# ka9q/ka9q-radio

Hardware: NVIDIA H100
Metric: input Msamples/s through forward+filter+inverse at N channels (higher is better)
Workload: dtype f32

## Files before the change

ka9q_radio_b200/csrc/fft_static.cuh:

```cuda
#pragma once
#include "fft_radix.cuh"

namespace kfft {

template <int LEN, int... RS> struct SPlan {
  static constexpr int len = LEN;
  static constexpr int nst = sizeof...(RS);
  static constexpr int rad_arr[sizeof...(RS) > 0 ? sizeof...(RS) : 1] = {RS...};
  static constexpr int rad(int i) { return rad_arr[i]; }
  static constexpr int nsub(int i) {
    int n = LEN;
    for (int k = 0; k < i; k++) n /= rad_arr[k];
    return n;
  }
  static constexpr int stride(int i) { return nsub(i) / rad_arr[i]; }
  static constexpr int tw_off(int i) {
    int o = 0;
    for (int k = 0; k < i; k++)
      if (stride(k) > 1) o += (rad_arr[k] - 1) * stride(k);
    return o;
  }
  static constexpr bool valid() {
    int p = 1;
    for (int k = 0; k < nst; k++) p *= rad_arr[k];
    return p == LEN;
  }
};

template <class P, int I = 0> struct SlotOf {
  static __device__ __forceinline__ int run(int rem) {
    constexpr int R = P::rad(I), S = P::stride(I);
    int const q = rem / R;
    return (rem - q * R) * S + SlotOf<P, I + 1>::run(q);
  }
};
template <class P> struct SlotOf<P, P::nst> {
  static __device__ __forceinline__ int run(int) { return 0; }
};
template <class P> __device__ __forceinline__ int static_slot(int k) { return SlotOf<P>::run(k); }

template <class P> constexpr int static_tw_count() { return P::tw_off(P::nst); }

__device__ __forceinline__ int ldg_stream_b32(int const *p) {
  int v;
  asm volatile("ld.global.nc.L1::no_allocate.b32 %0, [%1];" : "=r"(v) : "l"(p));
  return v;
}
__device__ __forceinline__ float2 ldg_stream_f2(float2 const *p) {
  float2 v;
  asm volatile("ld.global.nc.L1::no_allocate.v2.f32 {%0, %1}, [%2];" : "=f"(v.x), "=f"(v.y) : "l"(p));
  return v;
}

template <class P, int I> struct StageGeom {
  static constexpr int R = P::rad(I), NSUB = P::nsub(I), S = P::stride(I), NB = P::len / R;
  static __device__ __forceinline__ void split(int u, int &b, int &j) {
    if (S == 1) {
      b = u;
      j = 0;
    } else {
      b = u / S;
      j = u - b * S;
    }
  }
};

template <class P, bool INV, int I, bool TWS, int ILP>
__device__ __forceinline__ void static_stage(float2 *__restrict__ col, float2 const *__restrict__ tw, int lane) {
  using G = StageGeom<P, I>;
  constexpr int R = G::R, NSUB = G::NSUB, S = G::S, NB = G::NB, NL = 32;
  constexpr int ITERS = (NB + NL - 1) / NL;
  float2 const *twi = tw + P::tw_off(I);
#pragma unroll
  for (int it0 = 0; it0 < ITERS; it0 += ILP) {
    float2 x[ILP][R];
    float2 *p[ILP];
    int jj[ILP];
    bool ok[ILP];
#pragma unroll
    for (int q = 0; q < ILP; q++) {
      int const u = lane + NL * (it0 + q);
      ok[q] = (it0 + q < ITERS) && ((NB % NL == 0) || it0 + q + 1 < ITERS || u < NB);
      int b, j;
      G::split(ok[q] ? u : 0, b, j);
      jj[q] = j;
      p[q] = col + b * NSUB + j;
      if (ok[q]) {
#pragma unroll
        for (int m = 0; m < R; m++) x[q][m] = p[q][m * S];
      }
    }
#pragma unroll
    for (int q = 0; q < ILP; q++) {
      if (ok[q]) {
        Dft<R, INV>::run(x[q]);
        if (S > 1) {
#pragma unroll
          for (int t = 1; t < R; t++) {
            float2 const w = TWS ? twi[(t - 1) * S + jj[q]] : __ldg(twi + (t - 1) * S + jj[q]);
            x[q][t] = INV ? cmulc(x[q][t], w) : cmul(x[q][t], w);
          }
        }
      }
    }
#pragma unroll
    for (int q = 0; q < ILP; q++) {
      if (ok[q]) {
#pragma unroll
        for (int t = 0; t < R; t++) p[q][t * S] = x[q][t];
      }
    }
  }
}

template <class P, bool INV, bool TWS = false, int ILP = 1, int I = 0> struct StaticFft {
  static __device__ __forceinline__ void run(float2 *col, float2 const *tw, int lane) {
    static_stage<P, INV, I, TWS, (P::rad(I) <= 12 ? ILP : 1)>(col, tw, lane);
    __syncwarp();
    StaticFft<P, INV, TWS, ILP, I + 1>::run(col, tw, lane);
  }
};
template <class P, bool INV, bool TWS, int ILP> struct StaticFft<P, INV, TWS, ILP, P::nst> {
  static __device__ __forceinline__ void run(float2 *, float2 const *, int) {}
};

__device__ __forceinline__ uint32_t smem_u32(void const *p) { return (uint32_t)__cvta_generic_to_shared(p); }
__device__ __forceinline__ void mbar_init(uint64_t *bar, int count) {
  asm volatile("mbarrier.init.shared::cta.b64 [%0], %1;" ::"r"(smem_u32(bar)), "r"(count));
}
__device__ __forceinline__ void mbar_fence_init() { asm volatile("fence.mbarrier_init.release.cluster;" ::: "memory"); }
__device__ __forceinline__ void mbar_expect_tx(uint64_t *bar, uint32_t bytes) {
  asm volatile("mbarrier.arrive.expect_tx.shared::cta.b64 _, [%0], %1;" ::"r"(smem_u32(bar)), "r"(bytes) : "memory");
}
__device__ __forceinline__ void bulk_g2s(void *dst, void const *src, uint32_t bytes, uint64_t *bar) {
  asm volatile("cp.async.bulk.shared::cluster.global.mbarrier::complete_tx::bytes [%0], [%1], %2, [%3];" ::"r"(smem_u32(dst)),
               "l"(src), "r"(bytes), "r"(smem_u32(bar))
               : "memory");
}
__device__ __forceinline__ void tensor_g2s_3d(void *dst, void const *map, int x, int y, int z, uint64_t *bar) {
  asm volatile("cp.async.bulk.tensor.3d.shared::cluster.global.tile.mbarrier::complete_tx::bytes [%0], [%1, {%2, %3, %4}], [%5];"
               ::"r"(smem_u32(dst)), "l"(map), "r"(x), "r"(y), "r"(z), "r"(smem_u32(bar))
               : "memory");
}
__device__ __forceinline__ void fence_proxy_async_global() { asm volatile("fence.proxy.async.global;" ::: "memory"); }
__device__ __forceinline__ void discard_l2_line(void *p) { asm volatile("discard.global.L2 [%0], 128;" ::"l"(p) : "memory"); }
__device__ __forceinline__ void mbar_wait(uint64_t *bar, uint32_t parity) {
  asm volatile(
      "{\n\t.reg .pred p;\n\t"
      "WAIT_%=:\n\t"
      "mbarrier.try_wait.parity.shared::cta.b64 p, [%0], %1;\n\t"
      "@p bra DONE_%=;\n\t"
      "bra WAIT_%=;\n\t"
      "DONE_%=:\n\t}" ::"r"(smem_u32(bar)),
      "r"(parity)
      : "memory");
}

}
```

ka9q_radio_b200/csrc/fwd_fused.cuh:

```cuda
#pragma once
#include "fwd_cols_r36.cuh"
#include "static_kernels_v2.cuh"

namespace kfft {

struct FusedShape {
  static constexpr int N1 = 1296, N2 = 1250;
  static constexpr int TILES = (N2 + 7) / 8;
  static constexpr int NC = (TILES + 1) / 2;
  static constexpr int NR = (N1 / 2 + 1 + RowsV2Shape<true>::IPC - 1) / RowsV2Shape<true>::IPC;
  static constexpr int T = 2 * ColsR36Shape::T;
  static constexpr int RT = RowsV2Shape<true>::T;
  static constexpr size_t smem = 2 * ColsR36Shape::smem > RowsV2Shape<true>::smem ? 2 * ColsR36Shape::smem : RowsV2Shape<true>::smem;
  static constexpr int DEFAULT_LEAD = 40;
  static_assert(ColsR36Shape::smem % 16 == 0, "the second tile's memory 16-byte aligned");
  static_assert(T % 32 == 0 && ColsR36Shape::T % 32 == 0 && RT % 32 == 0, "whole warps per tile and per R item");
};

enum FusedKind : int { kFusedCol = 0, kFusedRow = 1 };
struct FusedItem {
  int kind, blk, idx;
};

__host__ __device__ __forceinline__ FusedItem fused_item(int t, int nblocks, int lead) {
  using F = FusedShape;
  if (t < F::NC) return {kFusedCol, 0, t};
  t -= F::NC;
  int const b = t / (F::NR + F::NC), p = t - b * (F::NR + F::NC);
  if (b >= nblocks - 1) return {kFusedRow, nblocks - 1, t - (nblocks - 1) * (F::NR + F::NC)};
  if (p < lead) return {kFusedCol, b + 1, p};
  int const q = p - lead, m = F::NC - lead;
  if (q < 2 * m) return (q & 1) ? FusedItem{kFusedCol, b + 1, lead + q / 2} : FusedItem{kFusedRow, b, q / 2};
  return {kFusedRow, b, q - m};
}

struct FusedArgs {
  unsigned *ctr;
  int nblocks, lead;
  int discard;
};

__device__ __forceinline__ void red_release_gpu_add(unsigned *p, unsigned v) {
  asm volatile("red.release.gpu.global.add.u32 [%0], %1;" ::"l"(p), "r"(v) : "memory");
}
__device__ __forceinline__ unsigned ld_acquire_gpu(unsigned const *p) {
  unsigned v;
  asm volatile("ld.acquire.gpu.global.u32 %0, [%1];" : "=r"(v) : "l"(p) : "memory");
  return v;
}

template <int FMT>
__global__ void __launch_bounds__(FusedShape::T, 1)
    fwd_fused_r36_v2(Pass1Args const a1, ColsR36Tables const t1, Pass2Args const a2, FwdTables const t2, FusedArgs const f,
                     const __grid_constant__ CUtensorMap tmap) {
  using F = FusedShape;
  extern __shared__ __align__(16) unsigned char smem_raw[];
  __shared__ __align__(8) uint64_t bars[RowsV2Shape<true>::COLS];
  __shared__ __align__(8) uint64_t tbar[2];
  __shared__ int s_ticket;
  int const tid = threadIdx.x;
  if (tid == 0) s_ticket = (int)atomicAdd(f.ctr, 1u);
  __syncthreads();
  FusedItem const it = fused_item(s_ticket, f.nblocks, f.lead);
  if (it.kind == kFusedCol) {
    int const h = tid >= ColsR36Shape::T, tile = 2 * it.idx + h;
    if (tile < F::TILES)
      fwd_cols_r36_body<FMT, F::N2, true>(a1, t1, &tmap, smem_raw + h * ColsR36Shape::smem, tbar[h], tid - h * ColsR36Shape::T,
                                           tile * 8, it.blk, [h] {
                                             asm volatile("bar.sync %0, %1;" ::"r"(1 + h), "n"(ColsR36Shape::T) : "memory");
                                           });
    __syncthreads();
    if (tid == 0) {
      __threadfence();
      red_release_gpu_add(f.ctr + 1 + fused_item(s_ticket, f.nblocks, f.lead).blk, 1u);
    }
    return;
  }
  if (tid >= F::RT) return;
  auto sync = [] { asm volatile("bar.sync 3, %0;" ::"n"(F::RT) : "memory"); };
  auto sync_or = [](int p) {
    int r;
    asm volatile("{\n\t.reg .pred q, o;\n\tsetp.ne.s32 q, %1, 0;\n\tbar.red.or.pred o, 3, %2, q;\n\tselp.s32 %0, 1, 0, o;\n\t}"
                 : "=r"(r)
                 : "r"(p), "n"(F::RT)
                 : "memory");
    return r;
  };
  if (tid == 0)
    while (ld_acquire_gpu(f.ctr + 1 + it.blk) < (unsigned)F::NC) __nanosleep(64);
  sync();
  fwd_rows_v2_body<true, F::N1, true, true>(a2, t2, smem_raw, bars, tbar[0], tid, it.blk, it.idx * RowsV2Shape<true>::IPC,
                                            sync, sync_or, f.discard);
}

}
```

ka9q_radio_b200/csrc/static_kernels_v2.cuh:

```cuda
#pragma once
#include "static_kernels.cuh"

namespace kfft {

__device__ __forceinline__ void unpack_i16(int raw, int &lo, int &hi) {
  asm("prmt.b32 %0, %1, 0, 0x9910;" : "=r"(lo) : "r"(raw));
  hi = raw >> 16;
}
__device__ __forceinline__ float i32_to_f32(int v) {
  float f;
  asm("cvt.rn.f32.s32 %0, %1;" : "=f"(f) : "r"(v));
  return f;
}

template <bool REAL_SPLIT>
struct RowsV2Shape {
  using P = SPlan<1250, 10, 25, 5>;
  static constexpr int N2 = 1250, PITCH = 1250, GT = 256, SKEW = 2;
  static constexpr int NG = REAL_SPLIT ? 2 : 1, T = GT * NG, COLS = 8 * NG;
  static constexpr int IPC = REAL_SPLIT ? COLS / 2 : COLS;
  static constexpr int TW = (static_tw_count<P>() + 1) & ~1;
  static constexpr int TILE = COLS * PITCH + (NG - 1) * SKEW;
  static constexpr size_t smem = sizeof(float2) * (size_t)(TILE + TW);
  static __host__ __device__ constexpr int col_off(int c) { return c * PITCH + (c >> 3) * SKEW; }
};

__device__ constexpr float kRowsTw0[3][4][2] = {
    {{9.870916009e-01f, -1.601568460e-01f}, {9.486995935e-01f, -3.161789477e-01f}, {8.000617623e-01f, -5.999176502e-01f}, {2.801976204e-01f, -9.599423409e-01f}},
    {{9.486995935e-01f, -3.161789477e-01f}, {8.000617623e-01f, -5.999176502e-01f}, {2.801976204e-01f, -9.599423409e-01f}, {-8.429785967e-01f, -5.379471183e-01f}},
    {{8.858151436e-01f, -4.640382826e-01f}, {5.693368912e-01f, -8.221042752e-01f}, {-3.517109454e-01f, -9.361086488e-01f}, {-7.525988221e-01f, 6.584793329e-01f}},
};

__host__ __device__ constexpr int mid_row_lines(int mid_ld) { return mid_ld * 8 / 128; }
__host__ __device__ constexpr long mid_line(int blk, int n1, int row, int mid_ld, int l) {
  return ((long)blk * n1 + row) * mid_row_lines(mid_ld) + l;
}

template <bool REAL_SPLIT, int N1C, bool HALVED, bool FUSED, class Sync, class SyncOr>
__device__ __forceinline__ void fwd_rows_v2_body(Pass2Args const &a, FwdTables const &tb, unsigned char *smem_raw,
                                                 uint64_t *bars, uint64_t &tbar, int tid, int blk, int item0,
                                                 Sync const &sync, SyncOr const &sync_or, bool discard = false) {
  using S = RowsV2Shape<REAL_SPLIT>;
  using P = typename S::P;
  constexpr int N2 = S::N2, T = S::T, GT = S::GT, COLS = S::COLS, IPC = S::IPC;
  constexpr int R0 = 10, S0 = 125, R1 = 25, NSUB1 = 125, S1 = 5, R2 = 5;
  float2 *tile = reinterpret_cast<float2 *>(smem_raw);
  float2 *s_tw = tile + S::TILE;
  TilePlan const &pl = c_plans[a.plan];
  int const lane = tid & 31, warp = tid >> 5;
  int const n1 = N1C ? N1C : a.n1;
  auto row_of = [&](int col) -> int {
    RowItem const it = row_item(item0 + (REAL_SPLIT ? col >> 1 : col), n1, REAL_SPLIT);
    if (REAL_SPLIT) {
      if ((col & 1) == 0) return it.kind != kRowEmpty ? it.row_a : -1;
      return it.kind == kRowPair ? it.row_b : -1;
    }
    return it.kind == kRowPlain ? it.row_a : -1;
  };
  if (lane == 0) {
    int const row = row_of(warp);
    mbar_init(&bars[warp], 1);
    if (warp == 0) mbar_init(&tbar, 1);
    mbar_fence_init();
    if (row >= 0) {
      if (FUSED) fence_proxy_async_global();
      mbar_expect_tx(&bars[warp], N2 * 8);
      bulk_g2s(tile + S::col_off(warp), a.mid + ((long)blk * n1 + row) * a.mid_ld, N2 * 8, &bars[warp]);
    }
    if (warp == 0) {
      constexpr uint32_t TWB = (uint32_t)S::TW * 8u;
      mbar_expect_tx(&tbar, TWB);
      bulk_g2s(s_tw, pl.tw, TWB, &tbar);
    }
  }
  sync();
  int const g = tid / GT;
  int const c = (tid & 7) + 8 * g, ul = (tid % GT) >> 3;
  auto group_sync = [&] {
    if (S::NG == 1) sync();
    else asm volatile("bar.sync %0, %1;" ::"r"(1 + g), "n"(GT) : "memory");
  };
  bool const col_ok = row_of(c) >= 0;
  mbar_wait(&tbar, 0);
  if (col_ok) mbar_wait(&bars[c], 0);
  if (FUSED && discard && col_ok) {
    char *const mid = const_cast<char *>(reinterpret_cast<char const *>(a.mid));
    for (int l = ul; l < mid_row_lines(a.mid_ld); l += GT / 8) discard_l2_line(mid + 128 * mid_line(blk, n1, row_of(c), a.mid_ld, l));
  }
  float2 *mycol = tile + S::col_off(c);

  if (col_ok) {
    float2 base[4];
#pragma unroll
    for (int q = 0; q < 4; q++) base[q] = s_tw[((1 << q) - 1) * S0 + ul];
#pragma unroll
    for (int it = 0; it < 4; it++) {
      int const j = ul + (GT / 8) * it;
      if (it < 3 || j < S0) {
        float2 *p = mycol + j;
        float2 x[R0], w[R0];
#pragma unroll
        for (int m = 0; m < R0; m++) x[m] = p[m * S0];
#pragma unroll
        for (int q = 0; q < 4; q++)
          w[1 << q] = it == 0 ? base[q] : cmul(base[q], make_float2(kRowsTw0[it > 0 ? it - 1 : 0][q][0], kRowsTw0[it > 0 ? it - 1 : 0][q][1]));
        w[3] = cmul(w[2], w[1]);
        w[5] = cmul(w[4], w[1]);
        w[6] = cmul(w[4], w[2]);
        w[7] = cmul(w[4], w[3]);
        w[9] = cmul(w[8], w[1]);
        Dft<R0, false>::run(x);
        p[0] = x[0];
#pragma unroll
        for (int t = 1; t < R0; t++) p[t * S0] = cmul(x[t], w[t]);
      }
    }
  }
  group_sync();
  if (col_ok) {
    float2 const *tw1 = s_tw + P::tw_off(1);
#pragma unroll 1
    for (int u = ul; u < N2 / R1; u += GT / 8) {
      int const b = u / S1, j = u - b * S1;
      float2 *p = mycol + b * NSUB1 + j;
      float2 x[R1];
#pragma unroll
      for (int m = 0; m < R1; m++) x[m] = p[m * S1];
      Dft<R1, false>::run(x);
#pragma unroll
      for (int t = 1; t < R1; t++) x[t] = cmul(x[t], tw1[(t - 1) * S1 + j]);
#pragma unroll
      for (int t = 0; t < R1; t++) p[t * S1] = x[t];
    }
  }
  constexpr int UQ = T / IPC;
  int const i = tid % IPC, uq = tid / IPC;
  RowItem const it = row_item(item0 + i, n1, REAL_SPLIT);
  float2 rootC = make_float2(1.f, 0.f), rd[4];
  bool self_item = false;
  if (REAL_SPLIT) {
    self_item = it.kind == kRowSelf0 || it.kind == kRowSelfMid;
    if (it.kind == kRowPair) rootC = __ldg(tb.rootC + it.row_a);
#pragma unroll
    for (int q = 0; q < 4; q++) {
      int const u = uq + UQ * q;
      int const t0 = u / 25, t1 = u - t0 * 25;
      rd[q] = (it.kind == kRowPair && u < N2 / R2) ? __ldg(a.rootD + t0 + 10 * t1) : make_float2(1.f, 0.f);
    }
  }
  int const has_self = sync_or(self_item);

  float2 *spec = a.spec + (long)blk * a.spec_stride;
  float const hf = HALVED ? 1.0f : 0.5f;
  if (!REAL_SPLIT) {
    if (col_ok) {
      float2 *dst = spec + row_of(c);
#pragma unroll 1
      for (int u = ul; u < N2 / R2; u += GT / 8) {
        int const t0 = u / 25, t1 = u - t0 * 25;
        int const kb = t0 + 10 * t1;
        float2 const *p = mycol + u * R2;
        float2 x[R2];
#pragma unroll
        for (int m = 0; m < R2; m++) x[m] = p[m];
        Dft<R2, false>::run(x);
        float2 *d = dst + (long)n1 * kb;
#pragma unroll
        for (int t = 0; t < R2; t++) d[(long)n1 * 250 * t] = x[t];
      }
    }
    return;
  }
  int const nc = N1C ? N1C * N2 : (int)a.nc;
  if (it.kind == kRowPair) {
    float2 const *ca = tile + S::col_off(2 * i), *cb = tile + S::col_off(2 * i + 1);
#pragma unroll
    for (int q = 0; q < 4; q++) {
      int const u = uq + UQ * q;
      if (u >= N2 / R2) break;
      int const t0 = u / 25, t1 = u - t0 * 25;
      int const kb = t0 + 10 * t1;
      float2 const wkb = cmul(rootC, rd[q]);
      float2 za[R2], zb[R2];
      float2 const *pa = ca + u * R2, *pb = cb + (N2 / R2 - 1 - u) * R2;
      float2 *pk = spec + (it.row_a + n1 * kb), *pm = spec + (nc - it.row_a - n1 * kb);
#pragma unroll
      for (int m = 0; m < R2; m++) {
        za[m] = pa[m];
        zb[m] = pb[m];
      }
      Dft<R2, false>::run(za);
      Dft<R2, false>::run(zb);
#pragma unroll
      for (int t = 0; t < R2; t++) {
        float2 const A = za[t], B = zb[R2 - 1 - t];
        float2 const w = (t == 0) ? wkb : cmul(wkb, wroot<10>(t));
        float2 const E = HALVED ? make_float2(A.x + B.x, A.y - B.y) : make_float2(0.5f * (A.x + B.x), 0.5f * (A.y - B.y));
        float2 const O = HALVED ? make_float2(A.x - B.x, A.y + B.y) : make_float2(0.5f * (A.x - B.x), 0.5f * (A.y + B.y));
        float2 const Pp = cmul(w, O);
        pk[(long)n1 * 250 * t] = make_float2(E.x + Pp.y, E.y - Pp.x);
        pm[-(long)n1 * 250 * t] = make_float2(E.x - Pp.y, -(E.y + Pp.x));
      }
    }
  }
  if (!has_self) return;
  for (int s = 0; s < IPC; s++) {
    RowItem const its = row_item(item0 + s, n1, true);
    if (its.kind != kRowSelf0 && its.kind != kRowSelfMid) continue;
    float2 *col = tile + S::col_off(2 * s);
    for (int u = tid; u < N2 / R2; u += T) {
      float2 x[R2];
#pragma unroll
      for (int m = 0; m < R2; m++) x[m] = col[u * R2 + m];
      Dft<R2, false>::run(x);
#pragma unroll
      for (int m = 0; m < R2; m++) col[u * R2 + m] = x[m];
    }
  }
  sync();
  for (int s = 0; s < IPC; s++) {
    RowItem const its = row_item(item0 + s, n1, true);
    if (its.kind != kRowSelf0 && its.kind != kRowSelfMid) continue;
    float2 const *col = tile + S::col_off(2 * s);
    float2 const rC = __ldg(tb.rootC + its.row_a);
    bool const self0 = its.kind == kRowSelf0;
    int const kend = self0 ? N2 / 2 + 1 : (N2 + 1) / 2;
    for (int k2 = tid; k2 < kend; k2 += T) {
      int const k2m = self0 ? (k2 == 0 ? 0 : N2 - k2) : N2 - 1 - k2;
      float2 const A = col[static_slot<P>(k2)], B = col[static_slot<P>(k2m)];
      float2 const w = cmul(rC, __ldg(a.rootD + k2));
      float2 const E = make_float2(hf * (A.x + B.x), hf * (A.y - B.y));
      float2 const O = make_float2(hf * (A.x - B.x), hf * (A.y + B.y));
      float2 const Pp = cmul(w, O);
      int const k = its.row_a + n1 * k2;
      spec[k] = make_float2(E.x + Pp.y, E.y - Pp.x);
      if (nc - k != k) spec[nc - k] = make_float2(E.x - Pp.y, -(E.y + Pp.x));
    }
  }
}

template <bool REAL_SPLIT, int N1C = 0, bool HALVED = false>
__global__ void __launch_bounds__(RowsV2Shape<REAL_SPLIT>::T, REAL_SPLIT ? 1 : 2) fwd_rows_v2(Pass2Args const a, FwdTables const tb) {
  extern __shared__ __align__(16) unsigned char smem_raw[];
  __shared__ __align__(8) uint64_t bars[RowsV2Shape<REAL_SPLIT>::COLS];
  __shared__ __align__(8) uint64_t tbar;
  fwd_rows_v2_body<REAL_SPLIT, N1C, HALVED, false>(a, tb, smem_raw, bars, tbar, threadIdx.x, gridDim.y - 1 - blockIdx.y,
                                                   blockIdx.x * RowsV2Shape<REAL_SPLIT>::IPC, [] { __syncthreads(); },
                                                   [](int p) { return __syncthreads_or(p); });
}

template <class P, bool OSC = false>
__global__ void __launch_bounds__(kChanWarps * 32) chan_v2(ChanArgs const a) {
  static_assert(P::nst == 2, "two-stage plans only");
  __shared__ __align__(8) uint64_t bars[kChanWarps];
  __shared__ __align__(8) uint64_t tbar;
  using S = StaticChan<P>;
  constexpr int NS = S::NS, R0 = P::rad(0), R1 = P::rad(1), S0 = NS / R0;
  static_assert(S0 == R1, "plan shape");
  S s;
  if (!static_prologue<P>(a, bars, tbar, s)) return;
  ChanDesc const &d = s.d;
  float2 *col = s.col;
  int const lane = s.lane;
  mbar_wait(&tbar, 0);
  if (d.flags & kChanIsb) {
    for (int wp = lane; wp < NS; wp += 32) col[wp] = s.product(wp);
    __syncwarp();
    isb_fold_warp(col, NS, S::TOP, lane);
    static_stage<P, true, 0, true, 1>(col, s.s_tw, lane);
    __syncwarp();
  } else if (lane < S0) {
    float2 x[R0];
#pragma unroll
    for (int m = 0; m < R0; m++) x[m] = s.product(lane + S0 * m);
    Dft<R0, true>::run(x);
    col[lane] = x[0];
#pragma unroll
    for (int t = 1; t < R0; t++) col[lane + S0 * t] = cmulc(x[t], s.s_tw[(t - 1) * S0 + lane]);
  }
  __syncwarp();
  bool const osc = OSC && (d.flags & kChanOsc) != 0;
  float pw = 0.f;
  int const ci = chan_index(a, s.oi);
  if (lane < R0) {
    float2 x[R1];
#pragma unroll
    for (int m = 0; m < R1; m++) x[m] = col[R1 * lane + m];
    Dft<R1, true>::run(x);
    int const first = NS - d.olen;
    if (!OSC || !osc) {
#pragma unroll
      for (int t = 0; t < R1; t++) {
        int const n = lane + R0 * t;
        if (n >= first) s.dst[n - first] = x[t];
      }
    } else if (OSC) {
      ChanAux const ax = a.aux[ci];
      long const k = a.block0 + s.blk - ax.osc_epoch;
#pragma unroll
      for (int t = 0; t < R1; t++) {
        int const n = lane + R0 * t;
        if (n >= first) s.dst[n - first] = osc_sample(ax, k, d.olen, n - first, x[t], pw);
      }
    }
  }
  if (OSC && osc && a.power) {
    pw = warp_sum(pw);
    if (lane == 0) a.power[(long)s.blk * a.power_stride + ci] = pw / (float)d.olen;
  }
}

}
```

Baseline: 103,300.

## Read row inputs directly from global in first FFT stage instead of bulk-copying to shared

The rows kernel no longer issues per-warp cp.async.bulk copies of each mid-buffer row into shared memory with an mbarrier per column. Each warp now loads its row straight from global via __ldcg inside the first radix stage, waits on the twiddle barrier only after issuing those loads, and writes the stage result into the shared tile. This removes the per-column barriers, the proxy fence and one full shared-memory round trip. In exchange the loads are synchronous, strided global reads whose latency is no longer hidden by the async copy engine, and the work mapping for stage 0 moves from groups of eight threads per column to one warp per column.

```diff
diff --git a/ka9q_radio_b200/csrc/fft_static.cuh b/ka9q_radio_b200/csrc/fft_static.cuh
--- a/ka9q_radio_b200/csrc/fft_static.cuh
+++ b/ka9q_radio_b200/csrc/fft_static.cuh
@@ -142,7 +142,6 @@
                ::"r"(smem_u32(dst)), "l"(map), "r"(x), "r"(y), "r"(z), "r"(smem_u32(bar))
                : "memory");
 }
-__device__ __forceinline__ void fence_proxy_async_global() { asm volatile("fence.proxy.async.global;" ::: "memory"); }
 __device__ __forceinline__ void discard_l2_line(void *p) { asm volatile("discard.global.L2 [%0], 128;" ::"l"(p) : "memory"); }
 __device__ __forceinline__ void mbar_wait(uint64_t *bar, uint32_t parity) {
   asm volatile(
diff --git a/ka9q_radio_b200/csrc/fwd_fused.cuh b/ka9q_radio_b200/csrc/fwd_fused.cuh
--- a/ka9q_radio_b200/csrc/fwd_fused.cuh
+++ b/ka9q_radio_b200/csrc/fwd_fused.cuh
@@ -55,7 +55,6 @@
                      const __grid_constant__ CUtensorMap tmap) {
   using F = FusedShape;
   extern __shared__ __align__(16) unsigned char smem_raw[];
-  __shared__ __align__(8) uint64_t bars[RowsV2Shape<true>::COLS];
   __shared__ __align__(8) uint64_t tbar[2];
   __shared__ int s_ticket;
   int const tid = threadIdx.x;
@@ -89,7 +88,7 @@
   if (tid == 0)
     while (ld_acquire_gpu(f.ctr + 1 + it.blk) < (unsigned)F::NC) __nanosleep(64);
   sync();
-  fwd_rows_v2_body<true, F::N1, true, true>(a2, t2, smem_raw, bars, tbar[0], tid, it.blk, it.idx * RowsV2Shape<true>::IPC,
+  fwd_rows_v2_body<true, F::N1, true, true>(a2, t2, smem_raw, tbar[0], tid, it.blk, it.idx * RowsV2Shape<true>::IPC,
                                             sync, sync_or, f.discard);
 }
 
diff --git a/ka9q_radio_b200/csrc/static_kernels_v2.cuh b/ka9q_radio_b200/csrc/static_kernels_v2.cuh
--- a/ka9q_radio_b200/csrc/static_kernels_v2.cuh
+++ b/ka9q_radio_b200/csrc/static_kernels_v2.cuh
@@ -38,8 +38,8 @@
 
 template <bool REAL_SPLIT, int N1C, bool HALVED, bool FUSED, class Sync, class SyncOr>
 __device__ __forceinline__ void fwd_rows_v2_body(Pass2Args const &a, FwdTables const &tb, unsigned char *smem_raw,
-                                                 uint64_t *bars, uint64_t &tbar, int tid, int blk, int item0,
-                                                 Sync const &sync, SyncOr const &sync_or, bool discard = false) {
+                                                 uint64_t &tbar, int tid, int blk, int item0, Sync const &sync,
+                                                 SyncOr const &sync_or, bool discard = false) {
   using S = RowsV2Shape<REAL_SPLIT>;
   using P = typename S::P;
   constexpr int N2 = S::N2, T = S::T, GT = S::GT, COLS = S::COLS, IPC = S::IPC;
@@ -57,50 +57,37 @@
     }
     return it.kind == kRowPlain ? it.row_a : -1;
   };
-  if (lane == 0) {
-    int const row = row_of(warp);
-    mbar_init(&bars[warp], 1);
-    if (warp == 0) mbar_init(&tbar, 1);
+  if (tid == 0) {
+    constexpr uint32_t TWB = (uint32_t)S::TW * 8u;
+    mbar_init(&tbar, 1);
     mbar_fence_init();
-    if (row >= 0) {
-      if (FUSED) fence_proxy_async_global();
-      mbar_expect_tx(&bars[warp], N2 * 8);
-      bulk_g2s(tile + S::col_off(warp), a.mid + ((long)blk * n1 + row) * a.mid_ld, N2 * 8, &bars[warp]);
-    }
-    if (warp == 0) {
-      constexpr uint32_t TWB = (uint32_t)S::TW * 8u;
-      mbar_expect_tx(&tbar, TWB);
-      bulk_g2s(s_tw, pl.tw, TWB, &tbar);
-    }
+    mbar_expect_tx(&tbar, TWB);
+    bulk_g2s(s_tw, pl.tw, TWB, &tbar);
   }
   sync();
   int const g = tid / GT;
-  int const c = (tid & 7) + 8 * g, ul = (tid % GT) >> 3;
   auto group_sync = [&] {
     if (S::NG == 1) sync();
     else asm volatile("bar.sync %0, %1;" ::"r"(1 + g), "n"(GT) : "memory");
   };
-  bool const col_ok = row_of(c) >= 0;
-  mbar_wait(&tbar, 0);
-  if (col_ok) mbar_wait(&bars[c], 0);
-  if (FUSED && discard && col_ok) {
-    char *const mid = const_cast<char *>(reinterpret_cast<char const *>(a.mid));
-    for (int l = ul; l < mid_row_lines(a.mid_ld); l += GT / 8) discard_l2_line(mid + 128 * mid_line(blk, n1, row_of(c), a.mid_ld, l));
-  }
-  float2 *mycol = tile + S::col_off(c);
-
-  if (col_ok) {
+
+  int const row0 = row_of(warp);
+  if (row0 >= 0) {
+    float2 const *src = a.mid + ((long)blk * n1 + row0) * a.mid_ld;
+    float2 *const col0 = tile + S::col_off(warp);
     float2 base[4];
 #pragma unroll
-    for (int q = 0; q < 4; q++) base[q] = s_tw[((1 << q) - 1) * S0 + ul];
-#pragma unroll
     for (int it = 0; it < 4; it++) {
-      int const j = ul + (GT / 8) * it;
+      int const j = lane + 32 * it;
       if (it < 3 || j < S0) {
-        float2 *p = mycol + j;
         float2 x[R0], w[R0];
 #pragma unroll
-        for (int m = 0; m < R0; m++) x[m] = p[m * S0];
+        for (int m = 0; m < R0; m++) x[m] = __ldcg(src + j + m * S0);
+        if (it == 0) {
+          mbar_wait(&tbar, 0);
+#pragma unroll
+          for (int q = 0; q < 4; q++) base[q] = s_tw[((1 << q) - 1) * S0 + lane];
+        }
 #pragma unroll
         for (int q = 0; q < 4; q++)
           w[1 << q] = it == 0 ? base[q] : cmul(base[q], make_float2(kRowsTw0[it > 0 ? it - 1 : 0][q][0], kRowsTw0[it > 0 ? it - 1 : 0][q][1]));
@@ -110,13 +97,23 @@
         w[7] = cmul(w[4], w[3]);
         w[9] = cmul(w[8], w[1]);
         Dft<R0, false>::run(x);
+        float2 *p = col0 + j;
         p[0] = x[0];
 #pragma unroll
         for (int t = 1; t < R0; t++) p[t * S0] = cmul(x[t], w[t]);
       }
     }
+  } else {
+    mbar_wait(&tbar, 0);
   }
   group_sync();
+  if (FUSED && discard && row0 >= 0) {
+    char *const mid = const_cast<char *>(reinterpret_cast<char const *>(a.mid));
+    for (int l = lane; l < mid_row_lines(a.mid_ld); l += 32) discard_l2_line(mid + 128 * mid_line(blk, n1, row0, a.mid_ld, l));
+  }
+  int const c = (tid & 7) + 8 * g, ul = (tid % GT) >> 3;
+  bool const col_ok = row_of(c) >= 0;
+  float2 *mycol = tile + S::col_off(c);
   if (col_ok) {
     float2 const *tw1 = s_tw + P::tw_off(1);
 #pragma unroll 1
@@ -242,9 +239,8 @@
 template <bool REAL_SPLIT, int N1C = 0, bool HALVED = false>
 __global__ void __launch_bounds__(RowsV2Shape<REAL_SPLIT>::T, REAL_SPLIT ? 1 : 2) fwd_rows_v2(Pass2Args const a, FwdTables const tb) {
   extern __shared__ __align__(16) unsigned char smem_raw[];
-  __shared__ __align__(8) uint64_t bars[RowsV2Shape<REAL_SPLIT>::COLS];
   __shared__ __align__(8) uint64_t tbar;
-  fwd_rows_v2_body<REAL_SPLIT, N1C, HALVED, false>(a, tb, smem_raw, bars, tbar, threadIdx.x, gridDim.y - 1 - blockIdx.y,
+  fwd_rows_v2_body<REAL_SPLIT, N1C, HALVED, false>(a, tb, smem_raw, tbar, threadIdx.x, gridDim.y - 1 - blockIdx.y,
                                                    blockIdx.x * RowsV2Shape<REAL_SPLIT>::IPC, [] { __syncthreads(); },
                                                    [](int p) { return __syncthreads_or(p); });
 }
```

After: 103,000, median of 6. About the same (-0.3%).
